# LabJunBMI/E3-invaraint-diffusion-model

Measured on AMD Instinct MI355X. Metric: denoising-steps/sec (batched pocket graphs), higher is better.
Workload: dtype f32 storage and accumulation, f16x3 products (fp32 grade); 1 GPU; structure_model sampling step, 256 x 256-residue pockets per GPU, 12+12 layers x 768, T=1000 schedule, encoder recomputed every step (as the reference); pockets_per_gpu=256, seq_len=256, parallelism=pocket-sharded x1, no collective

## Files before the change

### e3-invaraint-diffusion-model_amd/bert.py

```python
from dataclasses import dataclass

import os

import torch
from torch import nn

from . import ops
from .autograd import functional as F


@dataclass
class BertConfig:
    hidden_size: int = 768
    num_attention_heads: int = 12
    intermediate_size: int = 1024
    num_hidden_layers: int = 12
    max_position_embeddings: int = 64
    position_embedding_type: str = "relative_key"
    hidden_dropout_prob: float = 0.1
    attention_probs_dropout_prob: float = 0.1
    layer_norm_eps: float = 1e-12
    hidden_act: str = "gelu"
    use_cache: bool = False
    is_decoder: bool = False
# ... 162 lines not shown


def _planes_for(att, x, drop):
    return (att.output.dense.weight, x) if drop[0] == 0 and drop[1] == 0 else None


def drop_keys(drop):
    return drop[2] if len(drop) > 2 else None


def run_self_attention(att, x, mask, B, L, drop=(0.0, 0.0), layout=None):
    sa = att.self
    w, b = qkv_weights(sa)
    qkv = F.linear(x, w, b, absmax=ops.absmax_slot(sa, "qkv", x.device))
    relkey = sa.position_embedding_type == "relative_key"
    if layout is not None:
        H = att.num_heads * 64
        ctx = ops.attention_varlen(qkv[:, :H], qkv[:, H:2 * H], qkv[:, 2 * H:], layout, layout, att.num_heads,
                                   dist_emb=sa.distance_embedding.weight if relkey else None,
                                   max_pos=sa.max_position_embeddings)
        return _attention_output(att, ctx, x)
    ctx = F.attention(qkv, None, B, att.num_heads, L, L, key_mask=mask,
                      dist_emb=sa.distance_embedding.weight if relkey else None,
                      max_pos=sa.max_position_embeddings, drop_p=drop[1], row_keys=drop_keys(drop),
                      planes_for=_planes_for(att, x, drop))
    return _attention_output(att, ctx, x, drop[0], drop_keys(drop))


def project_cross_kv(att, enc):
    w, b = kv_weights(att.self)
    return F.linear(enc, w, b, absmax=torch.zeros(1, device=enc.device, dtype=torch.float32))


def run_cross_attention(att, x, kv, enc_mask, B, Lq, Lk, drop=(0.0, 0.0), layout=None, enc_layout=None):
    q = F.linear(x, att.self.query.weight, att.self.query.bias, absmax=ops.absmax_slot(att.self, "q", x.device))
    if layout is not None:
        H = att.num_heads * 64
        ctx = ops.attention_varlen(q, kv[:, :H], kv[:, H:], layout, enc_layout, att.num_heads)
        return _attention_output(att, ctx, x)
    ctx = F.attention(q, kv, B, att.num_heads, Lq, Lk, key_mask=enc_mask, drop_p=drop[1], row_keys=drop_keys(drop),
                      planes_for=_planes_for(att, x, drop))
    return _attention_output(att, ctx, x, drop[0], drop_keys(drop))


def run_layer(layer, x, mask, B, L, cross_kv=None, enc_mask=None, Lk=None, drop=(0.0, 0.0), layout=None,
              enc_layout=None):
    x = run_self_attention(layer.attention, x, mask, B, L, drop, layout=layout)
    if hasattr(layer, "crossattention"):
        if cross_kv is None:
            raise ValueError("decoder layer needs encoder states")
        x = run_cross_attention(layer.crossattention, x, cross_kv, enc_mask, B, L, Lk, drop, layout=layout,
                                enc_layout=enc_layout)
    inter = F.linear(x, layer.intermediate.dense.weight, layer.intermediate.dense.bias, ops.ACT_GELU,
                     planes_for=(layer.output.dense.weight, x) if drop[0] == 0 and drop[1] == 0 else None)
    return F.linear_residual_layernorm(inter, layer.output.dense.weight, layer.output.dense.bias, x,
                                       layer.output.LayerNorm.weight, layer.output.LayerNorm.bias, layer.eps, drop[0],
                                       drop_keys(drop))


def run_encoder(encoder, x, mask, B, L, enc=None, enc_mask=None, Lk=None, cross_kv=None, layout=None, enc_layout=None,
                row_keys=None):
    drop = dropout_rates(encoder)
    if layout is not None and drop != (0.0, 0.0):
        raise RuntimeError("packed layouts are inference-only: put the model in eval mode")
    if row_keys is not None:
        drop = drop + (row_keys,)
    for i, layer in enumerate(encoder.layer):
        kv = None
        if hasattr(layer, "crossattention"):
            kv = cross_kv[i] if cross_kv is not None else project_cross_kv(layer.crossattention, enc)
        x = run_layer(layer, x, mask, B, L, kv, enc_mask, Lk, drop, layout=layout, enc_layout=enc_layout)
    return x
```

### e3-invaraint-diffusion-model_amd/csrc/gemm_split.hip

```cpp
#include <type_traits>

#include "e3d_common.h"

namespace {

typedef __bf16 bf16x8 __attribute__((ext_vector_type(8)));
typedef __bf16 bf16x4 __attribute__((ext_vector_type(4)));
typedef _Float16 f16x8 __attribute__((ext_vector_type(8)));
typedef _Float16 f16x4 __attribute__((ext_vector_type(4)));

template <typename E> struct Vec;
template <> struct Vec<__bf16> { typedef bf16x8 x8; typedef bf16x4 x4; };
template <> struct Vec<_Float16> { typedef f16x8 x8; typedef f16x4 x4; };
__device__ __forceinline__ f32x16 mma16(const bf16x8 a, const bf16x8 b, const f32x16 c) {
    return __builtin_amdgcn_mfma_f32_32x32x16_bf16(a, b, c, 0, 0, 0);
}
__device__ __forceinline__ f32x16 mma16(const f16x8 a, const f16x8 b, const f32x16 c) {
    return __builtin_amdgcn_mfma_f32_32x32x16_f16(a, b, c, 0, 0, 0);
}

struct Epi { float* absmax; float scale; int plan_m = 0; const int* run_if = nullptr; };

constexpr int BN = 128, BK = 32;
#ifdef GEMM_STAMPS
// ... 685 lines not shown
#pragma unroll
    for (int m = 0; m < 4; ++m) {
#pragma unroll
        for (int n = 0; n < 2; ++n) {
            const int col = col0 + wc * 64 + n * 32 + l31;
            const float bv = bias ? bias[col] : 0.f;
#pragma unroll
            for (int r = 0; r < 16; ++r) {
                const int row = row0 + wr * 128 + m * 32 + mfma32_row(r, half);
                float v = fmaf(acc[m][n][r], out_scale, bv);
                if (ACT == E3D_ACT_GELU) v = gelu_erf(v);
                if (ACT == E3D_ACT_SILU) v = silu(v);
                if (row < M) {
                    out[(int64_t)row * ldc + col] = v;
                    if (ACT == E3D_ACT_NONE && absmax) e3d_absmax_accum(amax, v);
                }
            }
        }
    }
    if (ACT == E3D_ACT_NONE && absmax) e3d_absmax_commit(amax, absmax, lane);
    STAMP_K(4);
#ifdef E3D_STAMPS
    asm volatile("s_waitcnt vmcnt(0)" ::: "memory");
    STAMP_K(5);
#endif
}

#ifdef E3D_NT_STORES
#define E3D_STORE_OUT(ptr, val) __builtin_nontemporal_store((val), (ptr))
#else
#define E3D_STORE_OUT(ptr, val) (*(ptr) = (val))
#endif

template <int ACT, typename E, bool PLANES = false>
__global__ __launch_bounds__(512, 2) void gemm_split256p_kernel(const float* __restrict__ A, int64_t lda,
                                                                 const float* __restrict__ W,
                                                                 const float* __restrict__ bias,
                                                                 float* __restrict__ out, int64_t ldc, int N, int K,
                                                                 int tiles_m, int tiles_n, float* __restrict__ absmax, float out_scale,
                                                                 const int* __restrict__ run_if) {
    if (run_if && *run_if == 0) return;
    extern __shared__ __attribute__((aligned(16))) unsigned char smem_raw[];
    constexpr int NS = 2, T_BYTES = BT * ROW64, BUF_BYTES = 2 * NS * T_BYTES;
    constexpr int NI = 8;
    const int total = tiles_m * tiles_n, nk = K / BK;
    const int tid = threadIdx.x, lane = tid & 63, wid = tid >> 6;
    const int wr = wid >> 2, wc = wid & 3;
    const int l31 = lane & 31, half = lane >> 5;

    unsigned goff[NI];
    int dst[NI];
#pragma unroll
    for (int i = 0; i < NI; ++i) {
        const int f = tid + 512 * (i & 3), r = f >> 3, kg = f & 7;
        goff[i] = (unsigned)(r * (i < 4 ? (int)lda : K) + kg * 4);
        dst[i] = (i < 4 ? 0 : NS * T_BYTES) + swz_off(r, kg >> 1) + (kg & 1) * 8;
    }

    int ld_tile = blockIdx.x, ld_k = 0;
    const float* ld_a;
    const float* ld_w;
    auto cursor_bases = [&]() {
        const int lid = xcd_remap(ld_tile, total);
        ld_a = A + (int64_t)(lid / tiles_n) * BT * lda + ld_k * BK;
        ld_w = W + (int64_t)(lid % tiles_n) * BT * K + ld_k * BK;
    };
    auto cursor_advance = [&]() {
        if (ld_k + 1 < nk) {
            ++ld_k;
            ld_a += BK;
            ld_w += BK;
        } else if (ld_tile + (int)gridDim.x < total) {
            ld_tile += gridDim.x;
            ld_k = 0;
            cursor_bases();
        }
    };
    f32x4 rg[NI];
    auto item_load = [&](int i) { rg[i] = *reinterpret_cast<const f32x4*>((i < 4 ? ld_a : ld_w) + goff[i]); };
    auto item_store = [&](int i, unsigned char* buf) {
        typename Vec<E>::x4 p[NS];
        split4<NS, E>(rg[i], p);
#pragma unroll
        for (int s = 0; s < NS; ++s) *reinterpret_cast<typename Vec<E>::x4*>(buf + s * T_BYTES + dst[i]) = p[s];
    };
    cursor_bases();
#pragma unroll
    for (int i = 0; i < NI; ++i) item_load(i);
    cursor_advance();
#pragma unroll
    for (int i = 0; i < NI; ++i) item_store(i, smem_raw);
#pragma unroll
    for (int i = 0; i < NI; ++i) item_load(i);
    cursor_advance();
    __syncthreads();

    int a_row[4], b_row[2];
#pragma unroll
// ... 74 lines not shown
                    asm volatile("" : "+v"(bl[r]));
                }
#pragma unroll
                for (int m = 0; m < 4; ++m) {
                    unsigned char* o = ob + ((int64_t)((row0 + wr * 128 + m * 32) >> 5) * nks + (colb >> 4)) * 2048;
#pragma unroll
                    for (int kl = 0; kl < 2; ++kl) {
                        f32x4 x0, x1;
#pragma unroll
                        for (int j = 0; j < 4; ++j) {
                            float a = fmaf(acc[m][n][8 * kl + j], out_scale, bl[8 * kl + j]);
                            float c = fmaf(acc[m][n][8 * kl + 4 + j], out_scale, bl[8 * kl + 4 + j]);
                            if (ACT == E3D_ACT_GELU) { a = gelu_erf(a); c = gelu_erf(c); }
                            if (ACT == E3D_ACT_SILU) { a = silu(a); c = silu(c); }
                            if (ACT == E3D_ACT_NONE && absmax) { e3d_absmax_accum(amax, a); e3d_absmax_accum(amax, c); }
                            asm volatile("" : "+v"(a));
                            asm volatile("" : "+v"(c));
                            const auto sw = __builtin_amdgcn_permlane32_swap(__float_as_uint(a), __float_as_uint(c), false, false);
                            x0[j] = __uint_as_float(sw[0]);
                            x1[j] = __uint_as_float(sw[1]);
                        }
                        typename Vec<E>::x4 p0[2], p1[2];
                        split4<2, E>(x0, p0);
                        split4<2, E>(x1, p1);
                        typedef typename Vec<E>::x8 X8;
                        *reinterpret_cast<X8*>(o + kl * 2048) = __builtin_shufflevector(p0[0], p1[0], 0, 1, 2, 3, 4, 5, 6, 7);
                        *reinterpret_cast<X8*>(o + kl * 2048 + 1024) = __builtin_shufflevector(p0[1], p1[1], 0, 1, 2, 3, 4, 5, 6, 7);
                    }
                }
            }
            continue;
        }
        const int lid = xcd_remap(tile, total);
        const int row0 = (lid / tiles_n) * BT, col0 = (lid % tiles_n) * BT;
#pragma unroll
        for (int m = 0; m < 4; ++m) {
#pragma unroll
            for (int n = 0; n < 2; ++n) {
                const int col = col0 + wc * 64 + n * 32 + l31;
                const float bv = bias ? bias[col] : 0.f;
                float* o = out + (int64_t)(row0 + wr * 128 + m * 32 + 4 * half) * ldc + col;
#pragma unroll
                for (int r = 0; r < 16; ++r) {
                    float v = fmaf(acc[m][n][r], out_scale, bv);
                    if (ACT == E3D_ACT_GELU) v = gelu_erf(v);
                    if (ACT == E3D_ACT_SILU) v = silu(v);
                    E3D_STORE_OUT(&o[(int64_t)((r & 3) + 8 * (r >> 2)) * ldc], v);
                    if (ACT == E3D_ACT_NONE && absmax) e3d_absmax_accum(amax, v);
                }
            }
        }
    }
    if (ACT == E3D_ACT_NONE && absmax) e3d_absmax_commit(amax, absmax, lane);
}

template <int ACT, typename E, bool PLANES = false>
int launch256p(const float* A, int64_t lda, const float* W, const float* bias, float* out, int64_t ldc, int M, int N,
               int K, Epi epi, hipStream_t s) {
    const int tiles_m = M / BT, tiles_n = N / BT;
    constexpr size_t lds = 2 * 2 * 2 * BT * ROW64;
    static std::atomic<uint64_t> lds_ok{0};
    const int n_cu = e3d_cu_count();
    const int total = tiles_m * tiles_n;
    e3d_allow_lds(lds_ok, gemm_split256p_kernel<ACT, E, PLANES>, lds);
    hipLaunchKernelGGL((gemm_split256p_kernel<ACT, E, PLANES>), dim3(total < n_cu ? total : n_cu), dim3(512), lds, s, A, lda, W, bias, out,
                       ldc, N, K, tiles_m, tiles_n, epi.absmax, epi.scale, epi.run_if);
    return e3d_launch_status(PLANES ? "e3d_gemm_bias_act_planes_split (persistent 256x256)" : "e3d_gemm_f32_split (persistent 256x256)");
}

int g_general_form = -1;
int g_tile_pref = -1;

template <int NS, int ACT, int WR, int WC, int NBUF, bool PIPE, typename E>
int launch256(const float* A, int64_t lda, const float* W, const float* bias, float* out, int64_t ldc, int M, int N,
              int K, Epi epi, hipStream_t s) {
    constexpr int TM = WR * 128, TN = WC * 64;
    const int tiles_m = (M + TM - 1) / TM, tiles_n = N / TN;
    const size_t lds = (size_t)NBUF * NS * (TM + TN) * ROW64;
    static std::atomic<uint64_t> lds_ok{0};
    e3d_allow_lds(lds_ok, gemm_split256_kernel<NS, ACT, WR, WC, NBUF, PIPE, E>, lds);
    hipLaunchKernelGGL((gemm_split256_kernel<NS, ACT, WR, WC, NBUF, PIPE, E>), dim3(tiles_m * tiles_n), dim3(WR * WC * 64), lds, s,
                       A, lda, W, bias, out, ldc, M, N, K, tiles_m, tiles_n, epi.absmax, epi.scale, epi.run_if);
    return e3d_launch_status("e3d_gemm_f32_split (128x64 wave tiles)");
}

template <int NS, int ACT, bool A_KMAJ, bool B_KMAJ, int WM, int WN, typename E, int TN = 2, bool TR = false>
int launch_general(const float* A, int64_t lda, const float* B, int64_t ldb, const float* bias, float* out, int64_t ldc,
                   int M, int N, int K, Epi epi, hipStream_t s);

int p_min() {
    static int v = 0;
    if (!v) {
        const char* e = getenv("E3D_GEMM_P_MIN");
        v = e ? atoi(e) : 160;
    }
    return v;
}

bool persistent_ok(int M, int Mp, int N, int K, int64_t lda, int64_t ldb, int k_min = 2 * BK) {
    if (g_tile_pref < 0) {
        const char* e = getenv("E3D_GEMM_TILE");
        g_tile_pref = e ? atoi(e) : 4;
    }
    const int64_t n_tiles = (int64_t)(Mp / BT) * (N / BT);
    return N % BT == 0 && M % BT == 0 && Mp % BT == 0 && ldb == K && g_tile_pref >= 4 && K >= k_min && lda < (1 << 22) &&
           (g_tile_pref >= 5 || n_tiles >= p_min() || (n_tiles >= 96 && N >= 6 * BT && !getenv("E3D_GEMM_P_MIN")));
}

template <int NS, int ACT, bool A_KMAJ, bool B_KMAJ, typename E>
int launch(const float* A, int64_t lda, const float* B, int64_t ldb, const float* bias, float* out, int64_t ldc,
           int M, int N, int K, Epi epi, hipStream_t s) {
    if (g_tile_pref < 0) {
        const char* e = getenv("E3D_GEMM_TILE");
        g_tile_pref = e ? atoi(e) : 4;
    }
    const int Mp = epi.plan_m > 0 ? epi.plan_m : M;
    if constexpr (!A_KMAJ && !B_KMAJ) {
        if constexpr (NS == 2) {
            if (persistent_ok(M, Mp, N, K, lda, ldb))
                return launch256p<ACT, E>(A, lda, B, bias, out, ldc, M, N, K, epi, s);
            if (N % BT == 0 && ldb == K && g_tile_pref >= 3 && (int64_t)((Mp + BT - 1) / BT) * (N / BT) >= 256)
                return launch256<NS, ACT, 2, 4, 2, true, E>(A, lda, B, bias, out, ldc, M, N, K, epi, s);
        }
        if constexpr (NS == 1) {
            if (N % BT == 0 && ldb == K && g_tile_pref >= 3 && (int64_t)((Mp + BT - 1) / BT) * (N / BT) >= 160)
                return launch256<NS, ACT, 2, 4, 2, true, E>(A, lda, B, bias, out, ldc, M, N, K, epi, s);
        }
        if (N % BT == 0 && ldb == K && g_tile_pref >= 1 &&
            (int64_t)((Mp + BT - 1) / BT) * (N / BT) >= 256)
            return launch256<NS, ACT, 2, 4, (NS <= 2 ? 2 : 1), false, E>(A, lda, B, bias, out, ldc, M, N, K, epi, s);
    }
    if (g_general_form < 0) {
        const char* e = getenv("E3D_GEMM_FORM");
        g_general_form = e ? atoi(e) : 0;
    }
    int form = g_general_form;
    if (form != 1 && form != 2 && form != 3 && form != 4) {
        const int64_t g256 = (int64_t)((Mp + 255) / 256) * ((N + 127) / 128), g128 = (int64_t)((Mp + 127) / 128) * ((N + 127) / 128);
        const int64_t cus = e3d_cu_count();
// ... 261 lines not shown

extern "C" int e3d_gemm_bias_act_f32_split_gated(const float* A, int64_t lda, const float* W, const float* bias, float* out,
                                                 int64_t ldc, int M, int N, int K, int act, int terms, float* out_absmax,
                                                 float out_scale, int plan_m, const int* run_if, void* stream) {
    E3D_REQUIRE(N % BN == 0, "gemm_split: need N%%128==0 (N=%d)", N);
    return gemm_split_general(A, lda, 0, W, (int64_t)K, 0, bias, out, ldc, M, N, K, act, terms, out_absmax, out_scale, stream,
                              plan_m, run_if);
}

extern "C" int e3d_gemm_planes_supported(int M, int N, int K, int64_t lda, int act, int terms) {
    return (terms == 3 || terms == E3D_TERMS_F16X3) && (act == E3D_ACT_NONE || act == E3D_ACT_GELU) && M > 0 && N > 0 && K > 0 &&
           K % BK == 0 && lda >= K && lda % 4 == 0 && persistent_ok(M, M, N, K, lda, K, BK);
}

extern "C" int e3d_gemm_bias_act_planes_split(const float* A, int64_t lda, const float* W, const float* bias, void* out_planes,
                                              int M, int N, int K, int act, int terms, float* out_absmax, float out_scale,
                                              void* stream) {
    E3D_REQUIRE(A && W && out_planes, "gemm_split (planes): null pointer");
    E3D_REQUIRE(e3d_gemm_planes_supported(M, N, K, lda, act, terms),
                "gemm_split (planes): this launch does not take the persistent kernel (M=%d N=%d K=%d act=%d terms=%d)", M, N, K, act, terms);
    E3D_REQUIRE(((uintptr_t)A % 16) == 0 && ((uintptr_t)W % 16) == 0 && ((uintptr_t)bias % 16) == 0 && ((uintptr_t)out_planes % 16) == 0,
                "gemm_split (planes): A, W, bias and the planes must be 16-byte aligned");
    E3D_REQUIRE(!out_absmax || act == E3D_ACT_NONE, "gemm_split (planes): out_absmax exists for act = none");
    const Epi epi{out_absmax, out_scale, 0, nullptr};
    hipStream_t s = (hipStream_t)stream;
    float* out = reinterpret_cast<float*>(out_planes);
    if (terms == 3) {
        if (act == E3D_ACT_GELU) return launch256p<E3D_ACT_GELU, __bf16, true>(A, lda, W, bias, out, N, M, N, K, epi, s);
        return launch256p<E3D_ACT_NONE, __bf16, true>(A, lda, W, bias, out, N, M, N, K, epi, s);
    }
    if (act == E3D_ACT_GELU) return launch256p<E3D_ACT_GELU, _Float16, true>(A, lda, W, bias, out, N, M, N, K, epi, s);
    return launch256p<E3D_ACT_NONE, _Float16, true>(A, lda, W, bias, out, N, M, N, K, epi, s);
}
```

### e3-invaraint-diffusion-model_amd/hip.py

```python
import ctypes
import os
from ctypes import c_char_p, c_float, c_int, c_int64, c_uint32, c_uint64, c_void_p

_HERE = os.path.dirname(os.path.abspath(__file__))
LIB_PATH = os.environ.get("E3D_HIP_LIB", os.path.join(_HERE, "libe3d_hip.so"))
ABI_VERSION = 5

_P = c_void_p
_VIEW = [_P, c_int64, c_int64]
_QKV = 3 * _VIEW + [_P, c_int, _P]
_SHAPE = 4 * [c_int]
_ATTN_FWD = _QKV + [_P, _P] + _SHAPE
_ATTN_BWD = _QKV + 3 * [_P] + 3 * _VIEW + [_P, _P] + _SHAPE
_STREAM = [_P]
_DROP = [c_float, c_uint64]
_DROP_KEYED = [c_float, c_uint32, _P]
_BOUNDS = [_P, c_int, _P, _P, _P]
_SIGNATURES = {
    "e3d_abi_version": (c_int, []),
    "e3d_last_error": (c_char_p, []),
    "e3d_gemm_bias_act_f32": (c_int, [_P, c_int64, _P, _P, _P, c_int64, c_int, c_int, c_int, c_int, _P]),
    "e3d_gemm_bias_act_f32_split": (c_int, [_P, c_int64, _P, _P, _P, c_int64, c_int, c_int, c_int, c_int, c_int, _P]),
    "e3d_gemm_bias_act_f32_split_ex": (c_int, [_P, c_int64, _P, _P, _P, c_int64, c_int, c_int, c_int, c_int, c_int, _P, c_float, _P]),
    "e3d_gemm_bias_act_f32_split_gated": (c_int, [_P, c_int64, _P, _P, _P, c_int64, c_int, c_int, c_int, c_int, c_int, _P, c_float,
# ... 7 lines not shown
    "e3d_gemm_skinny_plan_select": (None, [c_int, c_int]),
    "e3d_gemm_skinny_residual_layernorm_f32_split": (c_int, [_P, c_int64, _P, _P, _P, _P, _P, c_float, _P, c_int, c_int, c_int,
                                                     c_int, _P, c_int64, _P]),
    "e3d_gemm_skinny_residual_layernorm_f32_split_ex": (c_int, [_P, c_int64, _P, _P, _P, _P, _P, c_float, _P, c_int, c_int, c_int,
                                                        c_int, _P, c_int64, c_float, _P]),
    "e3d_attn_skip_padded_tiles": (c_int, [c_int]),
    "e3d_gemm_kernel_select": (c_int, [c_int]),
    "e3d_gemm_general_select": (c_int, [c_int]),
    "e3d_attn_rescale_tau": (c_float, [c_float]),
    "e3d_residual_layernorm_fwd": (c_int, [_P, _P, _P, _P, c_float, _P, _P, c_int, c_int, _P]),
    "e3d_adaln_gate_fwd": (c_int, [_P, _P, _P, c_int, c_int, _P, c_int, c_int, _P]),
    "e3d_embed_layernorm_fwd": (c_int, [_P, c_int, _P, _P, _P, _P, c_float, _P, c_int, _P, _P, c_int, c_int, _P]),
    "e3d_adaln_gate_indexed_fwd": (c_int, [_P, _P, _P, _P, c_int, _P, c_int, _P, c_int, c_int, _P]),
    "e3d_classify_onehot_rows": (c_int, [_P, c_int, _P, _P, c_int, _P]),
    "e3d_embed_layernorm_fwd_ex": (c_int, [_P, c_int, _P, _P, _P, _P, c_float, _P, c_int, _P, _P, c_int, c_int, _P, _P]),
    "e3d_nerf_backbone": (c_int, [_P, _P, _P, c_int, c_int, c_int, _P]),
    "e3d_gemm_f32_split_general": (c_int, [_P, c_int64, c_int, _P, c_int64, c_int, _P, _P, c_int64, c_int, c_int,
                                           c_int, c_int, c_int, _P]),
    "e3d_transpose_grouped_f32": (c_int, [_P, _P, c_int, c_int, c_int, c_int64, c_int64, _P]),
    "e3d_gemm_wgrad_grouped_f32_split": (c_int, [_P, _P, _P, _P, c_uint64, c_int, c_int64, c_int64, c_int, c_int, c_int, c_int, _P]),
    "e3d_residual_layernorm_drop_fwd": (c_int, [_P, _P, _P, _P, c_float, _P, _P, c_int, c_int, c_float, c_uint64, _P]),
    "e3d_layernorm_bwd_drop": (c_int, [_P, _P, _P, c_float, _P, _P, _P, _P, c_int, c_int, c_float, c_uint64, _P]),
    "e3d_weight_planes_bytes": (c_int64, [c_int, c_int]),
    "e3d_weight_planes_f32_split": (c_int, [_P, c_int, c_int, c_int, _P, _P]),
    "e3d_gemm_residual_layernorm_supported": (c_int, [c_int, c_int, c_int, c_int64]),
    "e3d_gemm_residual_layernorm_f32_split": (c_int, [_P, c_int64, _P, _P, _P, c_int64, _P, _P, c_float, _P, c_int64,
                                                      c_int, c_int, c_int, c_int, c_float, _P]),
    "e3d_activation_planes_bytes": (c_int64, [c_int, c_int]),
    "e3d_activation_planes_f32_split": (c_int, [_P, c_int64, c_int, c_int, c_int, _P, _P]),
    "e3d_gemm_residual_layernorm_planes_split": (c_int, [_P, _P, _P, _P, c_int64, _P, _P, c_float, _P, c_int64,
                                                         c_int, c_int, c_int, c_int, c_float, _P]),
    "e3d_gemm_planes_supported": (c_int, [c_int, c_int, c_int, c_int64, c_int, c_int]),
    "e3d_gemm_bias_act_planes_split": (c_int, [_P, c_int64, _P, _P, _P, c_int, c_int, c_int, c_int, c_int, _P, c_float, _P]),
    "e3d_attn_planes_supported": (c_int, [c_int64, c_int64, c_int64, c_int, c_int, c_int, c_int]),
    "e3d_relkey_attn_fwd_split_planes": (c_int, _QKV + [_P] + _SHAPE + [c_int] + _BOUNDS + _STREAM),
    "e3d_gemm_wgrad_ragged_f32_split": (c_int, [_P, _P, _P, _P, _P, _P, _P, _P, c_uint64, c_int, c_int, c_int, _P]),
    "e3d_relkey_attn_bwd_workspace_floats": (c_int64, [c_int, c_int, c_int, c_int, c_int]),
    "e3d_relkey_attn_bwd": (c_int, _ATTN_BWD + _STREAM),
    "e3d_dropout_f32": (c_int, [_P, c_float, c_uint64, _P, c_int64, _P]),
    "e3d_relkey_attn_fwd_split_drop": (c_int, _ATTN_FWD + [c_int] + _DROP + _STREAM),
    "e3d_relkey_attn_fwd_split_ex": (c_int, _ATTN_FWD + [c_int] + _DROP + _BOUNDS + _STREAM),
    "e3d_attn_scratch_bytes": (c_int64, [c_int]),
    "e3d_ddpm_step_wrap_table": (c_int, [_P, _P, _P, _P, _P, c_int, _P, c_int64, _P]),
    "e3d_relkey_attn_bwd_drop": (c_int, _ATTN_BWD + _DROP + _STREAM),
    "e3d_relkey_attn_bwd_ex": (c_int, _ATTN_BWD + [c_int] + _DROP + _STREAM),
    "e3d_attn_dropout_mask": (c_int, [c_int, c_int, c_int, c_int, c_float, c_uint64, _P, _P]),
    "e3d_layernorm_bwd": (c_int, [_P, _P, _P, c_float, _P, _P, _P, c_int, c_int, _P]),
    "e3d_layernorm_bwd_workspace_floats": (c_int64, [c_int, c_int]),
    "e3d_layernorm_bwd_ws": (c_int, [_P, _P, _P, c_float, _P, _P, _P, _P, c_int, c_int, c_float, c_uint64, _P, c_int64, _P]),
    "e3d_adaln_gate_bwd": (c_int, [_P, _P, _P, c_int, c_int, _P, _P, c_int, c_int, _P]),
    "e3d_act_fwd": (c_int, [_P, c_int, _P, c_int64, _P]),
    "e3d_act_bwd": (c_int, [_P, _P, c_int, _P, c_int64, _P]),
    "e3d_colsum": (c_int, [_P, c_int64, _P, c_int, c_int, _P]),
    "e3d_group_sum": (c_int, [_P, c_int, _P, c_int, c_int, _P]),
    "e3d_small_k_wgrad": (c_int, [_P, _P, _P, _P, c_int, c_int, c_int, c_int, _P]),
    "e3d_head_linear_bwd_dx": (c_int, [_P, _P, _P, c_int, c_int, c_int, _P]),
    "e3d_head_linear_fwd": (c_int, [_P, _P, _P, _P, c_int, c_int, c_int, _P]),
    "e3d_ddpm_step_wrap": (c_int, [_P, _P, _P, c_float, c_float, c_float, c_float, c_int, _P, c_int64, _P]),
    "e3d_q_sample_wrap": (c_int, [_P, _P, _P, _P, _P, _P, c_int, c_int64, _P]),
    "e3d_discrete_posterior_sample": (c_int, [_P, _P, _P, _P, _P, c_int, _P, _P, c_int, c_int, c_int, _P]),
    "e3d_discrete_q_sample": (c_int, [_P, _P, _P, c_int, _P, c_int, c_int, c_int, _P]),
    "e3d_optim_chunk_elems": (c_int, []),
    "e3d_grad_global_norm": (c_int, [_P, _P, _P, _P, c_int, c_float, _P, _P, _P]),
    "e3d_adamw_step_dyn": (c_int, [_P, _P, _P, _P, _P, _P, _P, c_int, _P, _P, c_float, c_float, c_float, c_float, _P]),
    "e3d_adamw_step_dev": (c_int, [_P, _P, _P, _P, _P, _P, _P, c_int, _P, _P, _P]),
    "e3d_dropout_set_epoch_ptr": (c_int, [_P]),
# ... 66 lines not shown
```

### e3-invaraint-diffusion-model_amd/ops.py

```python
import contextlib
import math
import os
import warnings

import torch

from . import hip, keyed

ACT_NONE, ACT_GELU, ACT_SILU = 0, 1, 2


def _stream():
    return torch.cuda.current_stream().cuda_stream


TRACE = None


_ROCTX = None


def _roctx():
    global _ROCTX
    if _ROCTX is None:
        _ROCTX = False
        if os.environ.get("E3D_ROCTX") == "1":
            import ctypes
            for name in ("libroctx64.so", "libroctx64.so.4", "/opt/rocm/lib/libroctx64.so"):
                try:
                    lib = ctypes.CDLL(name)
                    lib.roctxRangePushA.argtypes = [ctypes.c_char_p]
                    _ROCTX = lib
                    break
# ... 200 lines not shown
    if out is None:
        out = torch.empty((M, N), device=a.device, dtype=torch.float32)
    assert out.dim() == 2 and out.stride(1) == 1 and out.shape == (M, N)
    if absmax is not None:
        _chk(absmax, "gemm.absmax")
        assert act == ACT_NONE and absmax.numel() == 1
    scale = 1.0
    if terms == 19 and prescale:
        weight, scale = f16_weight(weight)
    if plan_m is not None or run_if is not None:
        _chk(run_if, "gemm.run_if", torch.int32)
        plan_m = M if plan_m is None else plan_m
        if not gemm_is_tiled(plan_m, mode):
            raise ValueError(f"gemm: plan_m / run_if exist on the tiled split kernels only (plan_m={plan_m}, mode={mode or GEMM_MODE})")
        with _timed("gemm" if run_if is None else "gemm_gated", (M, N, K, act)):
            hip.check(hip.lib().e3d_gemm_bias_act_f32_split_gated(
                _p(a), a.stride(0), _p(weight), _p(bias), _p(out), out.stride(0), M, N, K, act, terms, _p(absmax), scale,
                plan_m, _p(run_if), _stream()), "e3d_gemm_bias_act_f32_split_gated")
        return out
    with _timed("gemm", (M, N, K, act)):
        if _skinny_ok(terms, M, N, K, a) and out.stride(0) % 4 == 0 and M <= min(SKINNY_MAX_M, SKINNY_GEMM_MAX_M):
            ws = _skinny_workspace(a.device, M, N, K)
            hip.check(hip.lib().e3d_gemm_skinny_f32_split_ex(_p(a), a.stride(0), _p(weight), _p(bias), _p(out), out.stride(0),
                                                             M, N, K, act, terms, _p(ws), ws.numel(), _p(absmax), scale, _stream()),
                      "e3d_gemm_skinny_f32_split_ex")
        elif terms == 0:
            hip.check(hip.lib().e3d_gemm_bias_act_f32(_p(a), a.stride(0), _p(weight), _p(bias), _p(out),
                                                      out.stride(0), M, N, K, act, _stream()), "e3d_gemm_bias_act_f32")
        else:
            hip.check(hip.lib().e3d_gemm_bias_act_f32_split_ex(
                _p(a), a.stride(0), _p(weight), _p(bias), _p(out), out.stride(0), M, N, K, act, terms, _p(absmax), scale,
                _stream()), "e3d_gemm_bias_act_f32_split_ex")
    return out


class arithmetic:

    def __init__(self, mode, respect_env=True):
        self.gemm = os.environ.get("E3D_GEMM_MODE", mode) if respect_env else mode
        self.attn = os.environ.get("E3D_ATTN_MODE", self.gemm) if respect_env else mode

    def __enter__(self):
        self.prev = (set_gemm_mode(self.gemm), set_attn_mode(self.attn))
        return self

    def __exit__(self, *exc):
        set_gemm_mode(self.prev[0])
        set_attn_mode(self.prev[1])


ATTN_MODE = os.environ.get("E3D_ATTN_MODE", GEMM_MODE)
if ATTN_MODE == "bf16":
    ATTN_MODE = "bf16x3"
if ATTN_MODE not in GEMM_MODES:
    raise ValueError(f"E3D_ATTN_MODE must be one of {sorted(GEMM_MODES)}, got {ATTN_MODE!r}")


def set_attn_mode(mode):
    global ATTN_MODE
    if mode not in GEMM_MODES:
        raise ValueError(f"attention mode must be one of {sorted(GEMM_MODES)}, got {mode!r}")
    if mode == "bf16":
        mode = "bf16x3"
    prev, ATTN_MODE = ATTN_MODE, mode
    return prev

# ... 784 lines not shown
```

### e3-invaraint-diffusion-model_amd/structure_model/model.py

```python
import functools
from typing import List

import torch
from torch import nn

from .. import bert, keyed, ops
from ..blocks import (BertEmbeddings, GaussianFourierProjection, KeyedDropoutSwitch, Predictor, SELayer, drop_row_keys,
                      flat2d, onehot_modulation, require_gpu)
from ..training import adamw
import os

from .utils import elementwise_form, radian_l1_loss, radian_smooth_l1_loss

MASKED_LOSS = os.environ.get("E3D_MASKED_LOSS", "1") == "1"


class ReceptorCache:

    def __init__(self, encoder_states, cross_kv, mask, B, L, layout=None):
        self.encoder_states, self.cross_kv, self.mask, self.B, self.L = encoder_states, cross_kv, mask, B, L
        self.layout = layout


class ConditionalBertForDiffusionBase(nn.Module):
    def __init__(self, encoder_config, decoder_config, feature_size: int) -> None:
        super().__init__()
        self.encoder_config = encoder_config
        self.decoder_config = decoder_config
        self.receptor_seq_emb = BertEmbeddings(20, encoder_config)
        self.receptor_angle_emb = BertEmbeddings(feature_size, encoder_config)
        self.receptor_emb = SELayer(encoder_config)
        self.encoder = bert.BertEncoder(encoder_config)
        self.ligand_angle_emb = BertEmbeddings(feature_size, decoder_config)
        self.timestep_projector = GaussianFourierProjection(decoder_config.hidden_size)
        self.timestep_emb = SELayer(decoder_config)
        self.decoder = bert.BertEncoder(decoder_config)
        self.angles_predictor = Predictor(decoder_config.hidden_size, feature_size)

    def encode_receptor(self, receptor_seq, receptor_angles, receptor_attention_masks,
                        project_cross_kv=True, layout=None) -> ReceptorCache:
        require_gpu(receptor_seq, receptor_angles, receptor_attention_masks)
        B, L = receptor_angles.shape[:2]
        ops.reset_absmax(receptor_angles.device)
        if layout is not None:
            ang = self.receptor_angle_emb.run(flat2d(layout.pack(receptor_angles)))
            seq2d = flat2d(layout.pack(receptor_seq))
            mod = onehot_modulation(self.receptor_emb, self.receptor_seq_emb, seq2d)
            seq = self.receptor_seq_emb.run(seq2d) if mod is None else None
            x = self.receptor_emb.run(ang, seq, None, 1, layout.rows, mod=mod, layout=layout)
            x = bert.run_encoder(self.encoder, x, None, 1, layout.rows, layout=layout)
            kv = [bert.project_cross_kv(layer.crossattention, x) for layer in self.decoder.layer] if project_cross_kv else None
            return ReceptorCache(x, kv, None, B, L, layout=layout)
        mask = receptor_attention_masks.contiguous().float()
        rk = drop_row_keys(keyed.DROP_POCKET, L)
        ang = self.receptor_angle_emb.run(flat2d(receptor_angles), row_keys=rk)
        seq2d = flat2d(receptor_seq)
        mod = onehot_modulation(self.receptor_emb, self.receptor_seq_emb, seq2d)
        seq = self.receptor_seq_emb.run(seq2d, row_keys=rk) if mod is None else None
        x = self.receptor_emb.run(ang, seq, mask, B, L, mod=mod, row_keys=rk)
        x = bert.run_encoder(self.encoder, x, mask, B, L, row_keys=rk)
        kv = None
        if project_cross_kv:
            kv = [bert.project_cross_kv(layer.crossattention, x) for layer in self.decoder.layer]
        return ReceptorCache(x, kv, mask, B, L)

    def timestep_modulation(self, timesteps):
        temb = self.timestep_projector(timesteps.reshape(-1)).contiguous()
        return self.timestep_emb.modulation(temb)

    def decode(self, timestep, noised_ligand_angles, ligand_attention_masks, receptor: ReceptorCache, mod=None,
               layout=None):
        if layout is not None:
            return self._decode_packed(timestep, noised_ligand_angles, receptor, mod, layout)
        require_gpu(timestep, noised_ligand_angles, ligand_attention_masks)
        B, L = noised_ligand_angles.shape[:2]
        mask = ligand_attention_masks.contiguous().float()
        lk = drop_row_keys(keyed.DROP_LIGAND, L)
        x = self.ligand_angle_emb.run(flat2d(noised_ligand_angles), row_keys=lk)
        if mod is None:
            mod = self.timestep_modulation(timestep.squeeze(dim=-1))
        x = self.timestep_emb.run(x, None, mask, B, L, mod=mod, row_keys=lk)
        x = bert.run_encoder(self.decoder, x, mask, B, L, enc=receptor.encoder_states,
                             enc_mask=receptor.mask, Lk=receptor.L, cross_kv=receptor.cross_kv, row_keys=lk)
        return self.angles_predictor.run(x).view(B, L, -1)

    def _decode_packed(self, timestep, x_packed, receptor, mod, layout):
        require_gpu(x_packed)
        if receptor.layout is None:
            raise ValueError("a packed decode needs the pocket packed as well: encode_receptor(..., layout=)")
        assert x_packed.dim() == 2 and x_packed.shape[0] == layout.rows, (tuple(x_packed.shape), layout.rows)
        if mod is None:
            t = timestep.reshape(-1)
            assert bool((t == t[0]).all()), "a packed batch shares one timestep"
            mod = self.timestep_modulation(t[:1])
        assert mod.shape[0] == 1, "a packed batch shares one timestep: mod must be one row [1,6H]"
        x = self.ligand_angle_emb.run(x_packed.contiguous().float())
# ... 102 lines not shown
```

### include/e3d_hip.h

```cpp
#ifndef E3D_HIP_H
#define E3D_HIP_H

#include <stdint.h>

#ifdef __cplusplus
extern "C" {
#endif

#define E3D_ABI_VERSION 5

#define E3D_TERMS_BF16 1
#define E3D_TERMS_BF16X3 3
#define E3D_TERMS_BF16X6 6
#define E3D_TERMS_F16X3 19

#define E3D_ACT_NONE 0
#define E3D_ACT_GELU 1
#define E3D_ACT_SILU 2

int e3d_abi_version(void);
const char* e3d_last_error(void);

int e3d_gemm_bias_act_f32(const float* A, int64_t lda, const float* W, const float* bias,
                          float* out, int64_t ldc, int M, int N, int K, int act, void* stream);
// ... 221 lines not shown
int e3d_head_linear_bwd_dx(const float* dout, const float* W, float* dx, int M, int H, int Nout,
                           void* stream);

int e3d_residual_layernorm_drop_fwd(const float* x, const float* residual, const float* gamma, const float* beta, float eps,
                                    float* s_out, float* out, int M, int H, float drop_p, uint64_t drop_seed, void* stream);
int e3d_layernorm_bwd_drop(const float* dy, const float* s, const float* gamma, float eps, float* ds, float* ds_dropped,
                           float* dgamma, float* dbeta, int M, int H, float drop_p, uint64_t drop_seed, void* stream);
int64_t e3d_layernorm_bwd_workspace_floats(int M, int H);
int e3d_layernorm_bwd_ws(const float* dy, const float* s, const float* gamma, float eps, float* ds, float* ds_dropped,
                         float* dgamma, float* dbeta, int M, int H, float drop_p, uint64_t drop_seed, float* workspace,
                         int64_t workspace_floats, void* stream);

int64_t e3d_weight_planes_bytes(int N, int K);
int e3d_weight_planes_f32_split(const float* W, int N, int K, int terms, void* planes, void* stream);
int e3d_gemm_residual_layernorm_supported(int M, int N, int K, int64_t lda);
int e3d_gemm_residual_layernorm_f32_split(const float* A, int64_t lda, const void* w_planes, const float* bias,
                                          const float* residual, int64_t ldr, const float* gamma, const float* beta, float eps,
                                          float* out, int64_t ldo, int M, int N, int K, int terms, float out_scale, void* stream);

int64_t e3d_activation_planes_bytes(int M, int K);
int e3d_activation_planes_f32_split(const float* X, int64_t ldx, int M, int K, int terms, void* planes, void* stream);
int e3d_gemm_residual_layernorm_planes_split(const void* a_planes, const void* w_planes, const float* bias,
                                             const float* residual, int64_t ldr, const float* gamma, const float* beta, float eps,
                                             float* out, int64_t ldo, int M, int N, int K, int terms, float out_scale, void* stream);
int e3d_gemm_planes_supported(int M, int N, int K, int64_t lda, int act, int terms);
int e3d_gemm_bias_act_planes_split(const float* A, int64_t lda, const float* W, const float* bias, void* out_planes,
                                   int M, int N, int K, int act, int terms, float* out_absmax, float out_scale, void* stream);
int e3d_attn_planes_supported(int64_t k_rs, int64_t v_bs, int64_t v_rs, int Lq, int Lk, int terms, int have_scratch);
int e3d_relkey_attn_fwd_split_planes(const float* q, int64_t q_bs, int64_t q_rs, const float* k, int64_t k_bs,
                                     int64_t k_rs, const float* v, int64_t v_bs, int64_t v_rs,
                                     const float* dist_emb, int P, const float* key_mask, void* out_planes,
                                     int B, int nh, int Lq, int Lk, int terms, void* e_scratch, int e_scratch_ready,
                                     const float* q_absmax, const float* k_absmax, float* e_absmax, void* stream);

int e3d_adamw_step_dyn(float* const* params, const float* const* grads, float* const* exp_avg, float* const* exp_avg_sq,
                       const int64_t* numel, const int* chunk_tensor, const int64_t* chunk_first, int n_chunks,
                       const float* norm_and_clip, const float* lr_and_step, float beta1, float beta2, float eps,
                       float weight_decay, void* stream);
int e3d_adamw_step_dev(float* const* params, const float* const* grads, float* const* exp_avg, float* const* exp_avg_sq,
                       const int64_t* numel, const int* chunk_tensor, const int64_t* chunk_first, int n_chunks,
                       const float* norm_and_clip, const float* hyper, void* stream);
int e3d_dropout_set_epoch_ptr(const uint64_t* device_word);
int e3d_optim_chunk_elems(void);
int e3d_grad_global_norm(const float* const* grads, const int64_t* numel, const int* chunk_tensor, const int64_t* chunk_first,
                         int n_chunks, float max_norm, float* partial, float* norm_and_clip, void* stream);
int e3d_adamw_step(float* const* params, const float* const* grads, float* const* exp_avg, float* const* exp_avg_sq,
                   const int64_t* numel, const int* chunk_tensor, const int64_t* chunk_first, int n_chunks,
                   const float* norm_and_clip, float lr, float beta1, float beta2, float eps, float weight_decay, int step,
                   void* stream);

int e3d_adamw_ema_step(float* const* params, const float* const* grads, float* const* exp_avg, float* const* exp_avg_sq,
                       float* const* ema, const int64_t* numel, const int* chunk_tensor, const int64_t* chunk_first,
                       int n_chunks, const float* norm_and_clip, float lr, float beta1, float beta2, float eps,
                       float weight_decay, int step, float ema_decay, void* stream);
int e3d_adamw_ema_step_dev(float* const* params, const float* const* grads, float* const* exp_avg, float* const* exp_avg_sq,
                           float* const* ema, const int64_t* numel, const int* chunk_tensor, const int64_t* chunk_first,
                           int n_chunks, const float* norm_and_clip, const float* hyper, void* stream);

int e3d_keyed_drop_row_keys(const int64_t* ids, int B, int L, const int64_t* epoch_word, uint64_t seed, int stream,
                            uint64_t* out, void* st);
int e3d_dropout_f32_keyed(const float* x, float p, uint32_t site, const uint64_t* row_keys, float* out, int M, int H,
                          void* stream);
int e3d_keyed_attn_dropout_mask(int B, int nh, int Lq, int Lk, float p, uint32_t site, const uint64_t* row_keys, float* out,
                                void* stream);
int e3d_residual_layernorm_drop_fwd_keyed(const float* x, const float* residual, const float* gamma, const float* beta, float eps,
                                          float* s_out, float* out, int M, int H, float drop_p, uint32_t site,
// ... 44 lines not shown
```

Baseline: 4243 pocket-steps/s.

## Batch all decoder cross-attention K/V projections into one grouped persistent GEMM

Adds a grouped variant of the persistent 256x256 split-precision GEMM kernel. It takes a table of up to 16 weight/bias/output sets and spreads the tiles of every problem across one launch. The receptor path now projects K/V for all 12 decoder cross-attention layers from the shared encoder output in a single launch, replacing 12 separate launches. This cuts launch count and tail underutilisation, at the cost of per-tile table lookups, per-tile absmax atomics, and extra kernel instantiations.

```diff
diff --git a/e3-invaraint-diffusion-model_amd/bert.py b/e3-invaraint-diffusion-model_amd/bert.py
--- a/e3-invaraint-diffusion-model_amd/bert.py
+++ b/e3-invaraint-diffusion-model_amd/bert.py
@@ -218,6 +218,35 @@
     return F.linear(enc, w, b, absmax=torch.zeros(1, device=enc.device, dtype=torch.float32))
 
 
+def _cross_attentions(decoder):
+    return [layer.crossattention if hasattr(layer, "crossattention") else None for layer in decoder.layer]
+
+
+def cross_kv_is_grouped(decoder, enc):
+    atts = [att for att in _cross_attentions(decoder) if att is not None]
+    if not ops.GROUP_CROSS_KV or not atts or enc.dim() != 2:
+        return False
+    if torch.is_grad_enabled() and (enc.requires_grad or any(p.requires_grad for att in atts for p in att.self.parameters())):
+        return False
+    n_out = atts[0].self.key.weight.shape[0] + atts[0].self.value.weight.shape[0]
+    return (all(att.self.key.weight.shape == atts[0].self.key.weight.shape for att in atts)
+            and ops.gemm_is_persistent(enc, n_out))
+
+
+def project_all_cross_kv(decoder, enc):
+    atts = _cross_attentions(decoder)
+    if not cross_kv_is_grouped(decoder, enc):
+        return [None if att is None else project_cross_kv(att, enc) for att in atts]
+    kv = [None] * len(atts)
+    live = [i for i, att in enumerate(atts) if att is not None]
+    for c in range(0, len(live), ops.GEMM_GROUP_MAX):
+        part = live[c:c + ops.GEMM_GROUP_MAX]
+        packed = [kv_weights(atts[i].self) for i in part]
+        for i, o in zip(part, ops.gemm_grouped(enc, [w for w, _ in packed], [b for _, b in packed])):
+            kv[i] = o
+    return kv
+
+
 def run_cross_attention(att, x, kv, enc_mask, B, Lq, Lk, drop=(0.0, 0.0), layout=None, enc_layout=None):
     q = F.linear(x, att.self.query.weight, att.self.query.bias, absmax=ops.absmax_slot(att.self, "q", x.device))
     if layout is not None:
@@ -251,6 +280,8 @@
         raise RuntimeError("packed layouts are inference-only: put the model in eval mode")
     if row_keys is not None:
         drop = drop + (row_keys,)
+    if cross_kv is None and enc is not None and cross_kv_is_grouped(encoder, enc):
+        cross_kv = project_all_cross_kv(encoder, enc)
     for i, layer in enumerate(encoder.layer):
         kv = None
         if hasattr(layer, "crossattention"):
diff --git a/e3-invaraint-diffusion-model_amd/csrc/gemm_split.hip b/e3-invaraint-diffusion-model_amd/csrc/gemm_split.hip
--- a/e3-invaraint-diffusion-model_amd/csrc/gemm_split.hip
+++ b/e3-invaraint-diffusion-model_amd/csrc/gemm_split.hip
@@ -741,18 +741,54 @@
 #define E3D_STORE_OUT(ptr, val) (*(ptr) = (val))
 #endif
 
-template <int ACT, typename E, bool PLANES = false>
+constexpr int GEMM_GROUP_MAX = 16;
+struct GemmGroup {
+    const float* W[GEMM_GROUP_MAX];
+    const float* bias[GEMM_GROUP_MAX];
+    float* out[GEMM_GROUP_MAX];
+    float* absmax[GEMM_GROUP_MAX];
+    int64_t ldc[GEMM_GROUP_MAX];
+    float scale[GEMM_GROUP_MAX];
+    int count;
+};
+struct NoGroup {};
+__device__ __forceinline__ NoGroup group_table() { return {}; }
+__device__ __forceinline__ const GemmGroup& group_table(const GemmGroup& g) { return g; }
+
+__device__ __forceinline__ void absmax_raise(unsigned m, float* target, int lane) {
+#pragma unroll
+    for (int o = 32; o > 0; o >>= 1) {
+        const unsigned t = (unsigned)__shfl_xor((int)m, o, 64);
+        m = m > t ? m : t;
+    }
+    if (lane == 0) atomicMax(reinterpret_cast<unsigned*>(target), m);
+}
+
+template <int ACT, typename E, bool PLANES = false, typename... GT>
 __global__ __launch_bounds__(512, 2) void gemm_split256p_kernel(const float* __restrict__ A, int64_t lda,
                                                                  const float* __restrict__ W,
                                                                  const float* __restrict__ bias,
                                                                  float* __restrict__ out, int64_t ldc, int N, int K,
                                                                  int tiles_m, int tiles_n, float* __restrict__ absmax, float out_scale,
-                                                                 const int* __restrict__ run_if) {
+                                                                 const int* __restrict__ run_if, const GT... grps) {
     if (run_if && *run_if == 0) return;
     extern __shared__ __attribute__((aligned(16))) unsigned char smem_raw[];
+    constexpr bool GROUPED = sizeof...(GT) == 1;
+    static_assert(!GROUPED || (ACT == E3D_ACT_NONE && !PLANES), "the grouped launch exists for fp32 rows without activation");
+    const auto& grp = group_table(grps...);
     constexpr int NS = 2, T_BYTES = BT * ROW64, BUF_BYTES = 2 * NS * T_BYTES;
     constexpr int NI = 8;
-    const int total = tiles_m * tiles_n, nk = K / BK;
+    int groups = 1;
+    if constexpr (GROUPED) groups = grp.count;
+    const int total = tiles_m * tiles_n * groups, nk = K / BK;
+    auto group_tile = [&](int lid, int& rb, int& g, int& nb) {
+        if constexpr (GROUPED) {
+            g = lid / (tiles_m * tiles_n);
+            const int lo = lid - g * (tiles_m * tiles_n);
+            rb = lo / tiles_n;
+            nb = lo - rb * tiles_n;
+        }
+    };
     const int tid = threadIdx.x, lane = tid & 63, wid = tid >> 6;
     const int wr = wid >> 2, wc = wid & 3;
     const int l31 = lane & 31, half = lane >> 5;
@@ -771,8 +807,15 @@
     const float* ld_w;
     auto cursor_bases = [&]() {
         const int lid = xcd_remap(ld_tile, total);
-        ld_a = A + (int64_t)(lid / tiles_n) * BT * lda + ld_k * BK;
-        ld_w = W + (int64_t)(lid % tiles_n) * BT * K + ld_k * BK;
+        if constexpr (GROUPED) {
+            int rb, g, nb;
+            group_tile(lid, rb, g, nb);
+            ld_a = A + (int64_t)rb * BT * lda + ld_k * BK;
+            ld_w = grp.W[g] + (int64_t)nb * BT * K + ld_k * BK;
+        } else {
+            ld_a = A + (int64_t)(lid / tiles_n) * BT * lda + ld_k * BK;
+            ld_w = W + (int64_t)(lid % tiles_n) * BT * K + ld_k * BK;
+        }
     };
     auto cursor_advance = [&]() {
         if (ld_k + 1 < nk) {
@@ -913,7 +956,18 @@
             continue;
         }
         const int lid = xcd_remap(tile, total);
-        const int row0 = (lid / tiles_n) * BT, col0 = (lid % tiles_n) * BT;
+        int row0 = (lid / tiles_n) * BT, col0 = (lid % tiles_n) * BT;
+        if constexpr (GROUPED) {
+            int rb, g, nb;
+            group_tile(lid, rb, g, nb);
+            row0 = rb * BT;
+            col0 = nb * BT;
+            bias = grp.bias[g];
+            out = grp.out[g];
+            ldc = grp.ldc[g];
+            out_scale = grp.scale[g];
+            absmax = grp.absmax[g];
+        }
 #pragma unroll
         for (int m = 0; m < 4; ++m) {
 #pragma unroll
@@ -931,8 +985,14 @@
                 }
             }
         }
-    }
-    if (ACT == E3D_ACT_NONE && absmax) e3d_absmax_commit(amax, absmax, lane);
+        if constexpr (GROUPED) {
+            if (absmax) absmax_raise(amax, absmax, lane);
+            amax = 0;
+        }
+    }
+    if constexpr (!GROUPED) {
+        if (ACT == E3D_ACT_NONE && absmax) e3d_absmax_commit(amax, absmax, lane);
+    }
 }
 
 template <int ACT, typename E, bool PLANES = false>
@@ -978,14 +1038,14 @@
     return v;
 }
 
-bool persistent_ok(int M, int Mp, int N, int K, int64_t lda, int64_t ldb, int k_min = 2 * BK) {
+bool persistent_ok(int M, int Mp, int N, int K, int64_t lda, int64_t ldb, int k_min = 2 * BK, int groups = 1) {
     if (g_tile_pref < 0) {
         const char* e = getenv("E3D_GEMM_TILE");
         g_tile_pref = e ? atoi(e) : 4;
     }
-    const int64_t n_tiles = (int64_t)(Mp / BT) * (N / BT);
+    const int64_t n_tiles = (int64_t)(Mp / BT) * (N / BT) * groups;
     return N % BT == 0 && M % BT == 0 && Mp % BT == 0 && ldb == K && g_tile_pref >= 4 && K >= k_min && lda < (1 << 22) &&
-           (g_tile_pref >= 5 || n_tiles >= p_min() || (n_tiles >= 96 && N >= 6 * BT && !getenv("E3D_GEMM_P_MIN")));
+           (g_tile_pref >= 5 || n_tiles >= p_min() || (n_tiles >= 96 && (int64_t)N * groups >= 6 * BT && !getenv("E3D_GEMM_P_MIN")));
 }
 
 template <int NS, int ACT, bool A_KMAJ, bool B_KMAJ, typename E>
@@ -1313,3 +1373,45 @@
     if (act == E3D_ACT_GELU) return launch256p<E3D_ACT_GELU, _Float16, true>(A, lda, W, bias, out, N, M, N, K, epi, s);
     return launch256p<E3D_ACT_NONE, _Float16, true>(A, lda, W, bias, out, N, M, N, K, epi, s);
 }
+
+extern "C" int e3d_gemm_grouped_supported(int M, int N, int K, int64_t lda, int G) {
+    return G >= 1 && G <= GEMM_GROUP_MAX && M > 0 && N > 0 && K > 0 && K % BK == 0 && lda >= K && lda % 4 == 0 &&
+           (int64_t)(M / BT) * (N / BT) * G < (1ll << 30) && persistent_ok(M, M, N, K, lda, K, 2 * BK, G);
+}
+
+extern "C" int e3d_gemm_bias_f32_split_grouped(const float* A, int64_t lda, const float* const* W, int64_t ldb,
+                                               const float* const* bias, float* const* out, const int64_t* ldc,
+                                               const float* out_scale, float* const* out_absmax, int G, int M, int N, int K,
+                                               int terms, void* stream) {
+    E3D_REQUIRE(G >= 1 && G <= GEMM_GROUP_MAX, "gemm_split (grouped): 1..%d problems (G=%d)", GEMM_GROUP_MAX, G);
+    E3D_REQUIRE(A && W && out && ldc, "gemm_split (grouped): null pointer");
+    E3D_REQUIRE(terms == 3 || terms == E3D_TERMS_F16X3, "gemm_split (grouped): terms must be 3 or 19 (got %d)", terms);
+    E3D_REQUIRE(ldb == K, "gemm_split (grouped): weight rows must be contiguous (ldb=%lld, K=%d)", (long long)ldb, K);
+    E3D_REQUIRE(e3d_gemm_grouped_supported(M, N, K, lda, G),
+                "gemm_split (grouped): this launch does not take the persistent kernel (M=%d N=%d K=%d lda=%lld G=%d)", M, N, K,
+                (long long)lda, G);
+    E3D_REQUIRE(((uintptr_t)A % 16) == 0, "gemm_split (grouped): A must be 16-byte aligned");
+    GemmGroup g;
+    for (int p = 0; p < GEMM_GROUP_MAX; ++p) {
+        const int q = p < G ? p : 0;
+        E3D_REQUIRE(W[q] && out[q] && ((uintptr_t)W[q] % 16) == 0, "gemm_split (grouped): null or unaligned pointer in problem %d", q);
+        E3D_REQUIRE(ldc[q] >= N, "gemm_split (grouped): ldc=%lld < N=%d in problem %d", (long long)ldc[q], N, q);
+        g.W[p] = W[q]; g.bias[p] = bias ? bias[q] : nullptr; g.out[p] = out[q]; g.ldc[p] = ldc[q];
+        g.scale[p] = out_scale ? out_scale[q] : 1.0f;
+        g.absmax[p] = out_absmax ? out_absmax[q] : nullptr;
+    }
+    g.count = G;
+    const int tiles_m = M / BT, tiles_n = N / BT, total = tiles_m * tiles_n * G, n_cu = e3d_cu_count();
+    constexpr size_t lds = 2 * 2 * 2 * BT * ROW64;
+    hipStream_t s = (hipStream_t)stream;
+    const dim3 grid(total < n_cu ? total : n_cu), block(512);
+    static std::atomic<uint64_t> ok_bf16{0}, ok_f16{0};
+    auto go = [&](auto kern, std::atomic<uint64_t>& lds_ok) {
+        e3d_allow_lds(lds_ok, kern, lds);
+        hipLaunchKernelGGL(kern, grid, block, lds, s, A, lda, (const float*)nullptr, (const float*)nullptr, (float*)nullptr, (int64_t)0,
+                           N, K, tiles_m, tiles_n, (float*)nullptr, 1.0f, (const int*)nullptr, g);
+    };
+    if (terms == 3) go(gemm_split256p_kernel<E3D_ACT_NONE, __bf16, false, GemmGroup>, ok_bf16);
+    else go(gemm_split256p_kernel<E3D_ACT_NONE, _Float16, false, GemmGroup>, ok_f16);
+    return e3d_launch_status("e3d_gemm_bias_f32_split_grouped (persistent 256x256)");
+}
diff --git a/e3-invaraint-diffusion-model_amd/hip.py b/e3-invaraint-diffusion-model_amd/hip.py
--- a/e3-invaraint-diffusion-model_amd/hip.py
+++ b/e3-invaraint-diffusion-model_amd/hip.py
@@ -63,6 +63,8 @@
                                                          c_int, c_int, c_int, c_int, c_float, _P]),
     "e3d_gemm_planes_supported": (c_int, [c_int, c_int, c_int, c_int64, c_int, c_int]),
     "e3d_gemm_bias_act_planes_split": (c_int, [_P, c_int64, _P, _P, _P, c_int, c_int, c_int, c_int, c_int, _P, c_float, _P]),
+    "e3d_gemm_grouped_supported": (c_int, [c_int, c_int, c_int, c_int64, c_int]),
+    "e3d_gemm_bias_f32_split_grouped": (c_int, [_P, c_int64, _P, c_int64, _P, _P, _P, _P, _P, c_int, c_int, c_int, c_int, c_int, _P]),
     "e3d_attn_planes_supported": (c_int, [c_int64, c_int64, c_int64, c_int, c_int, c_int, c_int]),
     "e3d_relkey_attn_fwd_split_planes": (c_int, _QKV + [_P] + _SHAPE + [c_int] + _BOUNDS + _STREAM),
     "e3d_gemm_wgrad_ragged_f32_split": (c_int, [_P, _P, _P, _P, _P, _P, _P, _P, c_uint64, c_int, c_int, c_int, _P]),
diff --git a/e3-invaraint-diffusion-model_amd/ops.py b/e3-invaraint-diffusion-model_amd/ops.py
--- a/e3-invaraint-diffusion-model_amd/ops.py
+++ b/e3-invaraint-diffusion-model_amd/ops.py
@@ -1,4 +1,5 @@
 import contextlib
+import ctypes
 import math
 import os
 import warnings
@@ -265,6 +266,63 @@
                 _p(a), a.stride(0), _p(weight), _p(bias), _p(out), out.stride(0), M, N, K, act, terms, _p(absmax), scale,
                 _stream()), "e3d_gemm_bias_act_f32_split_ex")
     return out
+
+
+GROUP_CROSS_KV = os.environ.get("E3D_GROUP_CROSS_KV", "1") == "1"
+GEMM_GROUP_MAX = 16
+
+
+def gemm_grouped_ok(a, N, G, mode=None):
+    terms = GEMM_MODES[GEMM_MODE if mode is None else mode]
+    if terms not in (3, 19) or not 1 <= G <= GEMM_GROUP_MAX or a.dim() != 2 or a.stride(1) != 1:
+        return False
+    return bool(hip.lib().e3d_gemm_grouped_supported(a.shape[0], N, a.shape[1], a.stride(0), G))
+
+
+def gemm_is_persistent(a, N, mode=None):
+    terms = GEMM_MODES[GEMM_MODE if mode is None else mode]
+    M, K = a.shape
+    if _skinny_ok(terms, M, N, K, a) and M <= min(SKINNY_MAX_M, SKINNY_GEMM_MAX_M):
+        return False
+    return gemm_grouped_ok(a, N, 1, mode)
+
+
+def gemm_grouped(a, weights, biases, absmax=None, outs=None, mode=None):
+    G = len(weights)
+    _chk(a, "gemm_grouped.a")
+    assert a.dim() == 2 and a.stride(1) == 1 and len(biases) == G
+    M, K = a.shape
+    N = weights[0].shape[0] if G else 0
+    terms = GEMM_MODES[GEMM_MODE if mode is None else mode]
+    if absmax is None:
+        absmax = torch.zeros(max(G, 1), device=a.device, dtype=torch.float32)
+    _chk(absmax, "gemm_grouped.absmax")
+    assert absmax.dim() == 1 and absmax.numel() >= G and absmax.is_contiguous()
+    if outs is None:
+        outs = [torch.empty((M, N), device=a.device, dtype=torch.float32) for _ in range(G)]
+    n = max(G, 1)
+    a_w, a_b, a_o, a_m = ((ctypes.c_void_p * n)() for _ in range(4))
+    a_ldc, a_scale = (ctypes.c_int64 * n)(), (ctypes.c_float * n)()
+    keep = []
+    ldb = K
+    for g, (w, b, o) in enumerate(zip(weights, biases, outs)):
+        _chk(w, "gemm_grouped.weight"); _chk(b, "gemm_grouped.bias"); _chk(o, "gemm_grouped.out")
+        assert w.dim() == 2 and w.shape == (N, K) and w.stride(1) == 1, (tuple(w.shape), (N, K))
+        assert o.dim() == 2 and o.shape == (M, N) and o.stride(1) == 1
+        scale = 1.0
+        if w.stride(0) != K:
+            ldb = w.stride(0)
+        elif terms == 19:
+            w, scale = f16_weight(w)
+        keep.append(w)
+        a_w[g], a_b[g], a_o[g], a_m[g] = _p(w), _p(b), _p(o), absmax.data_ptr() + 4 * g
+        a_ldc[g], a_scale[g] = o.stride(0), scale
+    with _timed("gemm", (M, G * N, K, ACT_NONE, G)):
+        hip.check(hip.lib().e3d_gemm_bias_f32_split_grouped(_p(a), a.stride(0), a_w, ldb, a_b, a_o, a_ldc, a_scale, a_m, G, M, N, K,
+                                                            terms, _stream()), "e3d_gemm_bias_f32_split_grouped")
+    for g, o in enumerate(outs):
+        o._e3d_absmax = absmax[g:g + 1]
+    return outs
 
 
 class arithmetic:
diff --git a/e3-invaraint-diffusion-model_amd/structure_model/model.py b/e3-invaraint-diffusion-model_amd/structure_model/model.py
--- a/e3-invaraint-diffusion-model_amd/structure_model/model.py
+++ b/e3-invaraint-diffusion-model_amd/structure_model/model.py
@@ -49,7 +49,7 @@
             seq = self.receptor_seq_emb.run(seq2d) if mod is None else None
             x = self.receptor_emb.run(ang, seq, None, 1, layout.rows, mod=mod, layout=layout)
             x = bert.run_encoder(self.encoder, x, None, 1, layout.rows, layout=layout)
-            kv = [bert.project_cross_kv(layer.crossattention, x) for layer in self.decoder.layer] if project_cross_kv else None
+            kv = bert.project_all_cross_kv(self.decoder, x) if project_cross_kv else None
             return ReceptorCache(x, kv, None, B, L, layout=layout)
         mask = receptor_attention_masks.contiguous().float()
         rk = drop_row_keys(keyed.DROP_POCKET, L)
@@ -61,7 +61,7 @@
         x = bert.run_encoder(self.encoder, x, mask, B, L, row_keys=rk)
         kv = None
         if project_cross_kv:
-            kv = [bert.project_cross_kv(layer.crossattention, x) for layer in self.decoder.layer]
+            kv = bert.project_all_cross_kv(self.decoder, x)
         return ReceptorCache(x, kv, mask, B, L)
 
     def timestep_modulation(self, timesteps):
diff --git a/include/e3d_hip.h b/include/e3d_hip.h
--- a/include/e3d_hip.h
+++ b/include/e3d_hip.h
@@ -277,6 +277,11 @@
                                      const float* dist_emb, int P, const float* key_mask, void* out_planes,
                                      int B, int nh, int Lq, int Lk, int terms, void* e_scratch, int e_scratch_ready,
                                      const float* q_absmax, const float* k_absmax, float* e_absmax, void* stream);
+
+int e3d_gemm_grouped_supported(int M, int N, int K, int64_t lda, int G);
+int e3d_gemm_bias_f32_split_grouped(const float* A, int64_t lda, const float* const* W, int64_t ldb, const float* const* bias,
+                                    float* const* out, const int64_t* ldc, const float* out_scale, float* const* out_absmax,
+                                    int G, int M, int N, int K, int terms, void* stream);
 
 int e3d_adamw_step_dyn(float* const* params, const float* const* grads, float* const* exp_avg, float* const* exp_avg_sq,
                        const int64_t* numel, const int* chunk_tensor, const int64_t* chunk_first, int n_chunks,
```

Result: no change. 4252 pocket-steps/s, median of 6 (+0.2%).
